# eriq-augustine/KB2E

Measured on AMD Instinct MI355X. Metric: training triples/sec (1/2/4/8 MI355X) + FB15k Hits@10(Filter), higher is better.
Workload: dtype f64

## Files before the change

kb2e_amd/csrc/kernels_transr_pipe.hpp:

```cpp
#pragma once

#include "kernels_transr_cons.hpp"
#include "kernels_transr_seq.hpp"

namespace kb2e {

constexpr int kPipeList = 1536;

template <typename T>
__host__ __device__ constexpr size_t pipe_lds(int n) {
    return sizeof(T) * ((size_t)rm_np(n) * rm_ld(n) + 5 * (size_t)kChainRows * rm_ld(n) +
                        3 * (size_t)kChainRows * (kChainRows + 1) + 4 * kChainRows + 4 * (size_t)rm_np(n)) +
           sizeof(int) * (size_t)(2 * kPipeList + kSeqMaxTiles + 1 + 8 + 2 * kChainRows);
}

template <typename T, int KS>
__global__ __launch_bounds__(kChainThreads) void transr_cons_pipe_kernel(RParArgs a, RParBufs<T> bf) {
    using M = Mfma16<T>;
    static_assert(sizeof(T) == 8, "the D-row / k-step identity below is the FP64 fragment layout");
    constexpr int NB = (4 * KS + 15) / 16;
    constexpr int NP = 16 * NB, L = NP + 2, R = kChainRows, LG = R + 1;
    constexpr int NH = 2 * KS;
    constexpr int NSW = (NB + 2) / 3;
    static_assert(2 * R * L >= NP * L, "the K0 image borrows the two P buffers");
    static_assert(NSW * KS <= 4 * KS, "the helpers' slices share the walk's K0 registers");
    const int t0 = a.batch_t0[a.batch], t1 = a.batch_t0[a.batch + 1];
    int g0, r;
    if (!chain_first_tile(a, t0, t1, g0, r)) return;
    const int n = a.n, ld = a.ld;
    const int w = threadIdx.x >> 6, l = lane_id(), kq = l >> 4, l16 = l & 15;
    const bool mine = w < NB;
    const int col = 16 * w + l16;
    const int hw = w - 1;
    const T lr = (T)a.lr;
    extern __shared__ __attribute__((aligned(16))) char smem[];
    T* Wc = (T*)smem;
    T* Abuf = Wc + NP * L;
    T* Pbuf = Abuf + 3 * R * L;
    T* Gbuf = Pbuf + 2 * R * L;
    T* Cx = Gbuf + 2 * R * LG;
    T* qpart = Cx + R * LG;
    T* rp = qpart + 4 * R;
    int* pe = (int*)(rp + 4 * NP);
    int* ps = pe + kPipeList;
    int* pre = ps + kPipeList;
    int* misc = pre + kSeqMaxTiles + 1;
    int* vlist = misc + 8;
    const long long ck0 = clock64();
    unsigned long long n_chunks = 0, n_vio = 0, n_rounds = 0, max_m = 0;
    __shared__ unsigned long long ph[16];
    if (threadIdx.x < 16) ph[threadIdx.x] = 0;
    long long tq = ck0;
    auto tick = [&](int k) {
        if (bf.stats && threadIdx.x == (k >= 12 || k == 5 ? 64u : 0u)) {
            const long long t = clock64();
            ph[k] += (unsigned long long)(t - tq);
            tq = t;
        }
    };

    for (int idx = threadIdx.x; idx < NP * NP; idx += kChainThreads) {
        const int j = idx / NP, i = idx % NP;
        Wc[j * L + i] = (j < n && i < n) ? bf.W[((int64_t)r * n + j) * ld + i] : T(0);
    }
    if (w == 0) {
        int run = 0;
        for (int m0 = 0;; m0 += kWave) {
            const int g = g0 + m0 + l;
            const uint64_t b = __ballot(t0 + g < t1 && a.td_r[t0 + g] == r);
            const int k = b == ~0ull ? kWave : __builtin_ctzll(~b);
            run += k;
            if (k < kWave) break;
        }
        const int c0 = bf.cnrows[g0] & 127;
        const int rel = c0 > 0 && bf.cpairs[(int64_t)g0 * 2 * kCPairs + kCPairs + c0 - 1] == -2;
        int kl = -1, gt = -1;
        for (int g = g0 + run - 1; g >= g0 && kl < 0; --g) {
            const int cs = a.td_cnt[t0 + g] & 255;
            const int kk = l < cs ? a.td_kk[(t0 + g) * 8 + l] : -1;
            const uint64_t b = __ballot(kk >= 0 && a.act[kk]);
            if (b) {
                kl = __shfl(kk, 63 - __builtin_clzll(b));
                gt = g;
            }
        }
        int ntail = 0;
        if (gt >= 0) {
            const int cp = bf.cnrows[gt] & 127;
            const int sl = l < cp ? bf.cpairs[(int64_t)gt * 2 * kCPairs + kCPairs + l] : -3;
            ntail = __builtin_popcountll(__ballot(sl >= 0 && (sl >> 1) == kl * 2 + 1));
        }
        if (l == 0) {
            misc[3] = rel;
            misc[4] = gt;
            misc[5] = run;
            misc[6] = ntail;
        }
    }
    __syncthreads();
    const int run = misc[5], has_rel = misc[3], g_tail = misc[4], n_tail = misc[6];
    T reg[4 * KS];
    {
        T* K0 = Pbuf;
        if (mine) {
#pragma unroll
            for (int ib = 0; ib < NB; ++ib) {
                typename M::acc_t acc = {T(0), T(0), T(0), T(0)};
                T av[KS], bv[KS];
#pragma unroll
                for (int s = 0; s < KS; ++s) {
                    av[s] = Wc[(4 * s + kq) * L + ib * 16 + l16];
                    bv[s] = Wc[(4 * s + kq) * L + col];
                }
#pragma unroll
                for (int s = 0; s < KS; ++s) acc = M::mma(av[s], bv[s], acc);
#pragma unroll
                for (int qq = 0; qq < 4; ++qq) K0[(ib * 16 + kq + 4 * qq) * L + col] = acc[qq];
            }
        }
        __syncthreads();
        if (w == 0) {
            const int cK = l < NP ? l : 0;
#pragma unroll
            for (int i = 0; i < 4 * KS; ++i) reg[i] = K0[i * L + cK];
        } else {
#pragma unroll
            for (int i = 0; i < 4 * KS; ++i) reg[i] = T(0);
#pragma unroll
            for (int si = 0; si < NSW; ++si) {
                const int cb = hw + 3 * si;
                if (cb < NB) {
#pragma unroll
                    for (int s = 0; s < KS; ++s) reg[si * KS + s] = Wc[(4 * s + kq) * L + cb * 16 + l16];
                }
            }
        }
        if (threadIdx.x == 0) {
            misc[5] = 0;
            misc[6] = -1;
            misc[7] = -1;
        }
        __syncthreads();
    }
    bool changed = false;
    int32_t* const vio = bf.vio + (int64_t)g0 * kCPairs;
    int nvt = 0;
    int pend_nv = 0, pend_par = 0, pend_pc = 0, pend_ka = 0;
    tick(0);

    auto gram_tile = [&](const T* Ar, const T* Bm, int rt, int cb, T* out, int ldo) {
        typename M::acc_t acc = {T(0), T(0), T(0), T(0)};
        T av[KS], bv[KS];
#pragma unroll
        for (int s = 0; s < KS; ++s) {
            av[s] = Ar[(rt * 16 + l16) * L + 4 * s + kq];
            bv[s] = Bm[(cb * 16 + l16) * L + 4 * s + kq];
        }
#pragma unroll
        for (int s = 0; s < KS; ++s) acc = M::mma(av[s], bv[s], acc);
#pragma unroll
        for (int q = 0; q < 4; ++q) out[(rt * 16 + kq + 4 * q) * ldo + cb * 16 + l16] = acc[q];
    };
    auto proj_tile = [&](const T* Ar, int rt, int si, T* out) {
        const int cb = hw + 3 * si;
        typename M::acc_t acc = {T(0), T(0), T(0), T(0)};
        T av[KS];
#pragma unroll
        for (int s = 0; s < KS; ++s) av[s] = Ar[(rt * 16 + l16) * L + 4 * s + kq];
#pragma unroll
        for (int s = 0; s < KS; ++s) acc = M::mma(av[s], reg[si * KS + s], acc);
#pragma unroll
        for (int q = 0; q < 4; ++q) out[(rt * 16 + kq + 4 * q) * L + cb * 16 + l16] = acc[q];
    };
    constexpr int kHT = kChainThreads - kWave;
    constexpr int kRowsPer = (R * NP + kHT - 1) / kHT;
    static_assert(kRowsPer <= 32, "rows_ok bits");
    const int ht = (int)threadIdx.x - kWave;
    T rows[kRowsPer];
    uint32_t rows_ok = 0;
    auto load_rows = [&](int b, int e) {
        if (w == 0) return;
        int ent[kRowsPer];
#pragma unroll
        for (int q = 0; q < kRowsPer; ++q) {
            const int f = b + (ht + q * kHT) / NP;
            ent[q] = pe[f < kPipeList ? f : kPipeList - 1];
        }
        rows_ok = 0;
#pragma unroll
        for (int q = 0; q < kRowsPer; ++q) {
            const int idx = ht + q * kHT;
            const int k = idx / NP, j = idx % NP;
            const bool ok = idx < R * NP && b + k < e && ent[q] >= 0 && j < n;
            rows[q] = bf.ent[ok ? (uint32_t)ent[q] * (uint32_t)ld + (uint32_t)j : 0u];
            rows_ok |= (ok ? 1u : 0u) << q;
        }
    };
    auto store_rows = [&](int slot) {
        if (w == 0) return;
#pragma unroll
        for (int q = 0; q < kRowsPer; ++q) {
            const int idx = ht + q * kHT;
            if (idx < R * NP) Abuf[slot * R * L + (idx / NP) * L + idx % NP] = ((rows_ok >> q) & 1) ? rows[q] : T(0);
        }
    };
    int hsync_target = 0;
    auto helper_sync = [&]() {
        hsync_target += kChainThreads / kWave - 1;
        if (l == 0 && !((bf.dbg & 32) && hw == 0))
            __hip_atomic_fetch_add(&misc[5], 1, __ATOMIC_RELEASE, __HIP_MEMORY_SCOPE_WORKGROUP);
        for (uint32_t sp = 0;
             __hip_atomic_load(&misc[5], __ATOMIC_ACQUIRE, __HIP_MEMORY_SCOPE_WORKGROUP) < hsync_target; ++sp) {
            if (sp > (1u << 22)) {
                if (l == 0) __hip_atomic_store(bf.err, 1u, __ATOMIC_RELAXED, __HIP_MEMORY_SCOPE_AGENT);
                break;
            }
            __builtin_amdgcn_s_sleep(1);
        }
    };
    auto correct_inc = [&](T* Pn, int cn, const T* Pc, const T* An, const T* Ac, const int* vl, int ck) {
        constexpr int NE = NP / 16, NPS = (R + 11) / 12;
        const int rs = ht >> 4, cb = (ht & 15) * NE;
        T x[NPS][NE];
#pragma unroll
        for (int p = 0; p < NPS; ++p) {
            const int j = rs + 12 * p;
#pragma unroll
            for (int u = 0; u < NE; ++u) x[p][u] = j < cn ? Pn[j * L + cb + u] : T(0);
        }
        int used = 0;
        for (uint32_t sp = 0;; ++sp) {
            const bool done = __hip_atomic_load(&misc[6], __ATOMIC_ACQUIRE, __HIP_MEMORY_SCOPE_WORKGROUP) == ck;
            const int pw = __hip_atomic_load(&misc[7], __ATOMIC_ACQUIRE, __HIP_MEMORY_SCOPE_WORKGROUP);
            const int avail = (pw >> 6) == ck ? (pw & 63) : 0;
            for (; used < avail; ++used) {
                const int v = vl[used];
                T gv[NE], av[NE], d[NPS];
#pragma unroll
                for (int u = 0; u < NE; ++u) {
                    gv[u] = Pc[v * L + cb + u];
                    av[u] = Ac[v * L + cb + u];
                }
#pragma unroll
                for (int p = 0; p < NPS; ++p) {
                    const int j = rs + 12 * p;
                    d[p] = T(0);
#pragma unroll
                    for (int u = 0; u < NE; ++u) d[p] = fma(j < R ? An[j * L + cb + u] : T(0), av[u], d[p]);
                }
                row16_sums<T, NPS>(d);
#pragma unroll
                for (int p = 0; p < NPS; ++p) {
                    const int j = rs + 12 * p;
                    if (j < cn) {
                        const T gl = -lr * d[p];
#pragma unroll
                        for (int u = 0; u < NE; ++u) x[p][u] = fma(gl, gv[u], x[p][u]);
                    }
                }
            }
            if (done) break;
            if (sp > (1u << 22)) {
                if (l == 0) __hip_atomic_store(bf.err, 1u, __ATOMIC_RELAXED, __HIP_MEMORY_SCOPE_AGENT);
                break;
            }
            __builtin_amdgcn_s_sleep(1);
        }
        T sq[NPS];
#pragma unroll
        for (int p = 0; p < NPS; ++p) {
            const int j = rs + 12 * p;
            sq[p] = T(0);
            if (j < cn) {
#pragma unroll
                for (int u = 0; u < NE; ++u) {
                    if (used) Pn[j * L + cb + u] = x[p][u];
                    sq[p] = fma(x[p][u], x[p][u], sq[p]);
                }
            }
        }
        row16_sums<T, NPS>(sq);
        if ((ht & 15) == 0) {
#pragma unroll
            for (int p = 0; p < NPS; ++p) {
                const int j = rs + 12 * p;
                if (j < R) {
                    qpart[j] = j < cn ? sq[p] : T(0);
                    for (int v = 1; v < NB; ++v) qpart[v * R + j] = T(0);
                }
            }
        }
    };
    auto correct_q = [&](T* Pn, int cn, int nv, const T* Pc, const int* vl) {
        constexpr int NE = NP / 8;
        const int j = threadIdx.x >> 3, cb = (threadIdx.x & 7) * NE;
        T sq = T(0);
        if (j < cn) {
            T x[NE];
#pragma unroll
            for (int u = 0; u < NE; ++u) x[u] = Pn[j * L + cb + u];
            for (int k = 0; k < nv; ++k) {
                const int v = vl[k];
                const T gl = -lr * Cx[j * LG + v];
#pragma unroll
                for (int u = 0; u < NE; ++u) x[u] = fma(gl, Pc[v * L + cb + u], x[u]);
            }
#pragma unroll
            for (int u = 0; u < NE; ++u) {
                if (nv) Pn[j * L + cb + u] = x[u];
                sq = fma(x[u], x[u], sq);
            }
        }
        sq += dpp_mov<0xB1>(sq);
        sq += dpp_mov<0x4E>(sq);
        sq += dpp_mov<0x141>(sq);
        if ((threadIdx.x & 7) == 0) {
            qpart[j] = j < cn ? sq : T(0);
            for (int v = 1; v < NB; ++v) qpart[v * R + j] = T(0);
        }
    };
    auto apply_pending = [&]() {
        if (w == 0 || pend_nv == 0) return;
        const T* Pp = Pbuf + pend_pc * R * L;
        const T* Ap = Abuf + pend_ka * R * L;
        const int* vl = vlist + pend_par * R;
        const int vmine = l < pend_nv ? vl[l] : 0;
        T an[KS], gn[NSW];
        auto ldv = [&](int k) {
            const int v = __builtin_amdgcn_readlane(vmine, k);
#pragma unroll
            for (int s = 0; s < KS; ++s) an[s] = Ap[v * L + 4 * s + kq];
#pragma unroll
            for (int si = 0; si < NSW; ++si) {
                const int cb = hw + 3 * si;
                gn[si] = cb < NB ? -lr * Pp[v * L + cb * 16 + l16] : T(0);
            }
        };
        const int nvu = (bf.dbg & 16) ? 0 : pend_nv;
        if (nvu > 0) ldv(0);
        for (int k = 0; k < nvu; ++k) {
            T ac[KS], gc[NSW];
#pragma unroll
            for (int s = 0; s < KS; ++s) ac[s] = an[s];
#pragma unroll
            for (int si = 0; si < NSW; ++si) gc[si] = gn[si];
            if (k + 1 < nvu) ldv(k + 1);
#pragma unroll
            for (int si = 0; si < NSW; ++si)
                if (hw + 3 * si < NB) {
#pragma unroll
                    for (int s = 0; s < KS; ++s) reg[si * KS + s] = fma(ac[s], gc[si], reg[si * KS + s]);
                }
        }
    };
    auto renorm = [&] {
        if (w > 0) {
#pragma unroll
            for (int si = 0; si < NSW; ++si) {
                const int cb = hw + 3 * si;
#pragma unroll
                for (int s = 0; s < KS; ++s) {
                    T x[1] = {reg[si * KS + s] * reg[si * KS + s]};
                    row16_sums<T, 1>(x);
                    if (cb < NB && l16 == 0) rp[cb * NP + 4 * s + kq] = x[0];
                }
            }
        }
        __syncthreads();
        if (w > 0) {
#pragma unroll
            for (int si = 0; si < NSW; ++si) {
                if (hw + 3 * si >= NB) continue;
#pragma unroll
                for (int s = 0; s < KS; ++s) {
                    const int jr = 4 * s + kq;
                    T ss = rp[jr];
                    for (int v = 1; v < NB; ++v) ss += rp[v * NP + jr];
                    if (jr < n) reg[si * KS + s] = reg[si * KS + s] / sqrt(ss);
                }
            }
        }
        __syncthreads();
    };
    auto fresh = [&](const T* A, int cc, T* P, T* G) {
        const int nrt = cc > 16 ? 2 : 1;
        if (w > 0) {
#pragma unroll
            for (int si = 0; si < NSW; ++si)
                if (hw + 3 * si < NB)
                    for (int rt = 0; rt < nrt; ++rt) proj_tile(A, rt, si, P);
        } else {
            for (int gi = 0; gi < (nrt == 2 ? 3 : 1); ++gi) gram_tile(A, A, gi == 0 ? 0 : 1, gi == 2 ? 1 : 0, G, LG);
        }
        __syncthreads();
        correct_q(P, cc, 0, nullptr, vlist);
        __syncthreads();
    };

    const int tile_cap = bf.chain_tiles >= 1 && bf.chain_tiles < kSeqMaxTiles ? bf.chain_tiles : kSeqMaxTiles;
    const int list_cap = bf.chain_list >= 64 && bf.chain_list < kPipeList ? bf.chain_list : kPipeList;
    int pc = 0;
    int par = 0;
    for (int gw = g0; gw < g0 + run || gw == g0;) {
        if (w == 0) {
            const int nt = g0 + run - gw < tile_cap ? g0 + run - gw : tile_cap;
            int carry = 0, fit = 0;
            for (int m0 = 0; m0 < nt; m0 += kWave) {
                const int g = m0 + l;
                int c = g < nt ? (bf.cnrows[gw + g] & 127) : 0;
                if (gw + g == g0 && has_rel) c -= 1;
                int x = c;
#pragma unroll
                for (int s = 1; s < kWave; s <<= 1) {
                    const int y = __shfl_up(x, s);
                    if (l >= s) x += y;
                }
                if (g < nt) pre[g] = carry + x - c;
                fit += __builtin_popcountll(__ballot(g < nt && carry + x <= list_cap - 1));
                carry += __shfl(x, kWave - 1);
            }
            if (l == 0) {
                if (fit == nt) pre[nt] = carry;
                misc[0] = fit;
            }
        }
        __syncthreads();
        const int ntile = misc[0];
        const bool last = gw + ntile == g0 + run || (g_tail >= 0 && gw + ntile > g_tail);
        const int ntp = pre[ntile];
        const int npairs = ntp + (last && has_rel ? 1 : 0);
        const int tail_start = last && g_tail >= gw ? ntp - n_tail : npairs;
        for (int f = threadIdx.x; f < npairs; f += kChainThreads) {
            int e = r, sl = -2;
            if (f < ntp) {
                int lo = 0, hi = ntile - 1;
                while (lo < hi) {
                    const int mid = (lo + hi + 1) >> 1;
                    if (pre[mid] <= f) lo = mid;
                    else hi = mid - 1;
                }
                const int32_t* cp = bf.cpairs + (int64_t)(gw + lo) * 2 * kCPairs;
                e = cp[f - pre[lo]];
                sl = cp[kCPairs + f - pre[lo]];
            }
            pe[f] = e;
            ps[f] = sl;
        }
        auto chunk_end = [&](int b) {
            return b < tail_start ? (b + R < tail_start ? b + R : tail_start) : npairs;
        };
        __syncthreads();
        if (npairs > 0) {
            const int e0 = chunk_end(0);
            const int e1 = e0 < npairs ? chunk_end(e0) : e0;
            load_rows(0, e0);
            store_rows(0);
            load_rows(e0, e1);
            store_rows(1);
            load_rows(e1, e1 < npairs ? chunk_end(e1) : e1);
            if (tail_start == 0 && changed) renorm();
            __syncthreads();
            pc = 0;
            fresh(Abuf, e0, Pbuf, Gbuf);
        }
        int ka = 0;
        for (int base = 0; base < npairs;) {
            const int nbase = chunk_end(base);
            const int cc = nbase - base;
            const int nb2 = nbase < npairs ? chunk_end(nbase) : nbase;
            const int cn = nb2 - nbase;
            const T* A = Abuf + ka * R * L;
            const T* An = Abuf + (ka == 2 ? 0 : ka + 1) * R * L;
            T* P = Pbuf + pc * R * L;
            T* Pn = Pbuf + (pc ^ 1) * R * L;
            T* Gm = Gbuf + pc * R * LG;
            T* Gn = Gbuf + (pc ^ 1) * R * LG;
            int* vl = vlist + par * R;
            const int ck = (int)n_chunks;
            ++n_chunks;
            tick(1);
            if (w == 0) {
                const int j = l & (R - 1);
                T q = T(0);
                if (j < cc) {
                    q = qpart[j];
                    for (int v = 1; v < NB; ++v) q += qpart[v * R + j];
                }
                uint32_t vmask = 0;
                int npub = 0;
                if (__ballot(j < cc && q > T(1)) != 0) {
                    const T aaj = Gm[j * LG + j];
                    const int c0 = (l >> 5) * NH;
                    T x[NH];
#pragma unroll
                    for (int u = 0; u < NH; ++u) x[u] = P[j * L + c0 + u];
                    int cursor = 0;
                    const T eps = T(2) * lr;
                    for (;;) {
                        const uint64_t cand = __ballot(l < R && j < cc && j >= cursor && q > T(1));
                        if (!cand) break;
                        const int v = __builtin_ctzll(cand);
                        const int c = l;
                        const T pp = readlane_f(q, v);
                        const T aa = readlane_f(aaj, v);
                        const T cjv = Gm[j * LG + v];
                        const int slv = ps[base + v];
                        if (j == v) {
#pragma unroll
                            for (int u = 0; u < NH; ++u) P[v * L + c0 + u] = x[u];
                        }
                        tick(4);
                        const T pv = c < NP ? P[v * L + c] : T(0);
                        T vv4[4] = {T(0), T(0), T(0), T(0)};
#pragma unroll
                        for (int t = 0; t < KS; ++t)
#pragma unroll
                            for (int u = 0; u < 4; ++u) vv4[u] = fma(P[v * L + 4 * t + u], reg[4 * t + u], vv4[u]);
                        const T Vc = c < n ? (vv4[0] + vv4[1]) + (vv4[2] + vv4[3]) : T(0);
                        tick(7);
                        T s2[2] = {pv * Vc, Vc * Vc};
                        T rpp = __builtin_amdgcn_rcp(pp);
                        rpp = fma(fma(-pp, rpp, T(1)), rpp, rpp);
                        rpp = fma(fma(-pp, rpp, T(1)), rpp, rpp);
                        wave_sums<T, 2>(s2);
                        tick(8);
                        const T pV = s2[0], VV = s2[1];
                        const T pvd = pV + aa * pp, vvd = VV + T(2) * aa * pV + aa * aa * pp;
                        const T kappa = pvd * rpp;
                        const T w2t = vvd - kappa * pvd;
                        const T w2 = w2t > T(0) ? w2t : T(0);
                        const T rho = T(1) - eps * kappa;
                        T S0, S1;
                        const int m = transr_rounds_violator4(pp, w2, eps, rho, S0, S1);
                        n_rounds += (unsigned long long)m;
                        max_m = max_m > (unsigned long long)m ? max_m : (unsigned long long)m;
                        const T cpf = T(2) * (S0 + eps * S1 * kappa), cvf = T(2) * eps * S1;
                        const T g = c < n ? cpf * pv - cvf * (Vc + aa * pv) : T(0);
                        tick(9);
                        if (c < NP) P[v * L + c] = g;
                        {
                            T* dst = slv >= 0 ? bf.pair + (int64_t)slv * ld : bf.relpair + (int64_t)r * ld;
                            if (c < n) dst[c] = g;
                            if (l == 0) vio[nvt + npub] = slv;
                        }
                        tick(10);
                        const bool upd = j > v && j < cc;
                        T qh = T(0);
                        if (upd) {
                            const T gl = -lr * cjv;
                            T s4[4] = {T(0), T(0), T(0), T(0)};
#pragma unroll
                            for (int u = 0; u < NH; ++u) {
                                x[u] = fma(gl, P[v * L + c0 + u], x[u]);
                                s4[u & 3] = fma(x[u], x[u], s4[u & 3]);
                            }
                            qh = (s4[0] + s4[1]) + (s4[2] + s4[3]);
                        }
                        {
                            const T tot = pair_sum32(qh);
                            if (upd) q = tot;
                        }
                        if (l == 0) {
                            vl[npub] = v;
                            __hip_atomic_store(&misc[7], (ck << 6) | (npub + 1), __ATOMIC_RELEASE,
                                               __HIP_MEMORY_SCOPE_WORKGROUP);
                        }
                        ++npub;
                        vmask |= 1u << v;
                        cursor = v + 1;
                        ++n_vio;
                        tick(11);
                    }
                }
                if (l < cc) {
                    const int sl = ps[base + l];
                    const bool vio_l = (vmask >> l) & 1;
                    if (sl >= 0) bf.pflag[sl] = vio_l ? 1 : 0;
                    else if (vio_l) bf.relpair_stamp[r] = bf.stamp;
                }
                if (l == 0) {
                    misc[1 + 2 * par] = (int)vmask;
                    misc[2 + 2 * par] = npub;
                    __hip_atomic_store(&misc[6], ck, __ATOMIC_RELEASE, __HIP_MEMORY_SCOPE_WORKGROUP);
                }
                tick(2);
            } else {
                apply_pending();
                tick(12);
                if (cn > 0) {
                    const int nrt = cn > 16 ? 2 : 1, crt = cc > 16 ? 2 : 1;
#pragma unroll
                    for (int si = 0; si < NSW; ++si)
                        if (hw + 3 * si < NB)
                            for (int rt = 0; rt < nrt; ++rt) proj_tile(An, rt, si, Pn);
                    const int ng = nrt == 2 ? 3 : 1;
                    int load[3];
#pragma unroll
                    for (int h = 0; h < 3; ++h) load[h] = nrt * ((NB - h + 2) / 3);
                    for (int tl = 0; tl < ng; ++tl) {
                        int best = 0;
#pragma unroll
                        for (int h = 1; h < 3; ++h) best = load[h] < load[best] ? h : best;
                        ++load[best];
                        if (best == hw) gram_tile(An, An, tl == 0 ? 0 : 1, tl == 2 ? 1 : 0, Gn, LG);
                    }
                    (void)crt;
                }
                tick(13);
                helper_sync();
                tick(14);
                if (nb2 < npairs || cn > 0) {
                    store_rows(ka == 0 ? 2 : ka - 1);
                    const int n3 = nb2 < npairs ? chunk_end(nb2) : nb2;
                    load_rows(n3, n3 < npairs ? chunk_end(n3) : n3);
                }
                if (cn > 0) correct_inc(Pn, cn, P, An, A, vl, ck);
                tick(15);
            }
            __syncthreads();
            tick(w == 0 ? 3 : 5);
            const uint32_t vmask = (uint32_t)misc[1 + 2 * par];
            const int nv = misc[2 + 2 * par];
            pend_nv = nv;
            pend_par = par;
            pend_pc = pc;
            pend_ka = ka;
            nvt += nv;
            if (vmask) changed = true;
            const bool restart = nbase == tail_start && changed && cn > 0;
            tick(6);
            if (restart) {
                apply_pending();
                pend_nv = 0;
                __syncthreads();
                renorm();
                fresh(An, cn, Pn, Gn);
            }
            pc ^= 1;
            par ^= 1;
            ka = ka == 2 ? 0 : ka + 1;
            base = nbase;
        }
        apply_pending();
        pend_nv = 0;
        __syncthreads();
        gw += ntile;
        if (last || gw >= g0 + run) break;
    }
    if (w > 0) {
#pragma unroll
        for (int si = 0; si < NSW; ++si) {
            const int cb = hw + 3 * si;
            if (cb < NB) {
#pragma unroll
                for (int s = 0; s < KS; ++s) Wc[(4 * s + kq) * L + cb * 16 + l16] = reg[si * KS + s];
            }
        }
    }
    __syncthreads();
    if (mine && col < n)
        for (int jj = 0; jj < n; ++jj) bf.W[((int64_t)r * n + jj) * ld + col] = Wc[jj * L + col];
    chain_records<T, NP, L>(a, bf, r, vio, nvt, Wc, Pbuf, 2 * R * L);
    if (bf.stats) {
        if (threadIdx.x == 0) {
            const unsigned long long cyc = (unsigned long long)(clock64() - ck0);
            atomicAdd(&g_seq_stats[0], 1ull);
            atomicAdd(&g_seq_stats[1], n_chunks);
            atomicAdd(&g_seq_stats[2], n_vio);
            atomicAdd(&g_seq_stats[3], n_rounds);
            atomicAdd(&g_seq_stats[4], cyc);
            atomicMax(&g_seq_stats[5], cyc);
            atomicMax(&g_seq_stats[6], n_chunks);
            atomicMax(&g_seq_stats[7], max_m);
            for (int k = 0; k < 16; ++k) atomicAdd(&g_seq_stats[8 + k], ph[k]);
            if (n_chunks >= 20) {
                for (int k = 0; k < 16; ++k) atomicAdd(&g_seq_stats[24 + k], ph[k]);
                atomicAdd(&g_seq_stats[40], n_chunks);
                atomicAdd(&g_seq_stats[41], 1ull);
                atomicAdd(&g_seq_stats[42], n_vio);
            }
        }
    }
}

}
```

kb2e_amd/csrc/transr_cons.hip:

```cpp
#include "transr_cons.hpp"

#include <algorithm>
#include <cstring>
#include <stdexcept>
#include <string>
#include <utility>

#include "hip_util.hpp"
#include "kernels_transr_cons.hpp"
#include "kernels_transr_seq.hpp"
#include "kernels_transr_chainw.hpp"
#include "kernels_transr_chainwp.hpp"
#include "kernels_transr_chaing.hpp"
#include "kernels_transr_pipe.hpp"
#include "kernels_transr_wave.hpp"

namespace kb2e {

namespace {

enum Kind { kCons, kGrad, kProj };

int chain_grid(const RParArgs& a) { return a.nrel > 0 ? a.nrel : 1; }

template <typename T, int KS>
const void* fn_at(Kind k) {
    return k == kCons ? (const void*)transr_cons_wave_kernel<T, KS>
           : k == kGrad ? (const void*)transr_grad_wave_kernel<T, KS>
                        : (const void*)transr_proj_wave_kernel<T, KS>;
}

template <typename T, int... KS>
const void* fn_table(Kind k, int ks, std::integer_sequence<int, KS...>) {
    const void* tab[] = {fn_at<T, KS + 1>(k)...};
    return tab[ks - 1];
}

template <typename T>
const void* kernel_fn(Kind k, int n) {
    if (!cons_wave_supported(n)) throw std::runtime_error("TransR wave kernels: n > 64");
    return fn_table<T>(k, cons_live_steps<T>(n), std::make_integer_sequence<int, 16>{});
}

template <typename T>
const void* cons_fn(int n) {
    return kernel_fn<T>(kCons, n);
}

template <int... KS>
const void* pipe_table(int ks, std::integer_sequence<int, KS...>) {
    const void* tab[] = {(const void*)transr_cons_pipe_kernel<double, KS + 1>...};
    return tab[ks - 1];
}

const void* pipe_fn(int n) {
    if (!cons_wave_supported(n)) throw std::runtime_error("transRNorm pipelined chain kernel: n > 64");
    return pipe_table((n + 3) / 4, std::make_integer_sequence<int, 16>{});
}

const void* chainw_fn(int n) {
    switch (wide_nb(n)) {
        case 1: return (const void*)transr_cons_chain_wide_kernel<1>;
        case 2: return (const void*)transr_cons_chain_wide_kernel<2>;
        case 3: return (const void*)transr_cons_chain_wide_kernel<3>;
        case 4: return (const void*)transr_cons_chain_wide_kernel<4>;
        case 5: return (const void*)transr_cons_chain_wide_kernel<5>;
        case 6: return (const void*)transr_cons_chain_wide_kernel<6>;
        case 7: return (const void*)transr_cons_chain_wide_kernel<7>;
    }
    throw std::runtime_error("transRNorm wide chain kernel: n > 112");
}

const void* chainwp_fn(int n) {
    switch (wp_ks(n)) {
        case 18: return (const void*)transr_cons_chain_wpipe_kernel<18>;
        case 20: return (const void*)transr_cons_chain_wpipe_kernel<20>;
        case 22: return (const void*)transr_cons_chain_wpipe_kernel<22>;
        case 24: return (const void*)transr_cons_chain_wpipe_kernel<24>;
        case 25: return (const void*)transr_cons_chain_wpipe_kernel<25>;
    }
    throw std::runtime_error("transRNorm pipelined wide chain kernel: no instantiation");
}

bool use_wpipe(int n) {
    const char* e = getenv("KB2E_RPAR_CHAIN");
    return n > 64 && n <= kWPMaxN && !(e && std::string(e) == "lockstep");
}

}

size_t cons_seq_setup(int n) {
    const size_t lds = pipe_lds<double>(n);
    HIPCHK(hipFuncSetAttribute(pipe_fn(n), hipFuncAttributeMaxDynamicSharedMemorySize, (int)lds));
    return lds;
}

void cons_seq_launch(const RParArgs& a, const RParBufs<double>& bf, size_t lds, hipStream_t stream) {
    RParArgs aa = a;
    RParBufs<double> bb = bf;
    void* args[] = {&aa, &bb};
    HIPCHK(hipLaunchKernel(pipe_fn(a.n), dim3(chain_grid(a)), dim3(kChainThreads), args, lds, stream));
}

bool cons_chainw_supported(int n) { return n >= 1 && n <= kWideMaxN; }

size_t cons_chainw_setup(int n) {
    HIPCHK(hipFuncSetAttribute((const void*)transr_cons_da_rel_kernel, hipFuncAttributeMaxDynamicSharedMemorySize,
                               (int)da_rel_lds(n)));
    const bool wp = use_wpipe(n);
    const size_t lds = wp ? chainwp_lds(n) : chainw_lds(n);
    HIPCHK(hipFuncSetAttribute(wp ? chainwp_fn(n) : chainw_fn(n), hipFuncAttributeMaxDynamicSharedMemorySize,
                               (int)lds));
    return lds;
}

bool cons_chainw_pipelined(int n) { return use_wpipe(n); }

void cons_chainw_launch(const RParArgs& a, const RParBufs<double>& bf, size_t lds, hipStream_t stream) {
    RParArgs aa = a;
    RParBufs<double> bb = bf;
    void* args[] = {&aa, &bb};
    const int grid = chain_grid(a);
    if (use_wpipe(a.n)) {
        HIPCHK(hipLaunchKernel(chainwp_fn(a.n), dim3(grid), dim3(kWPThreads), args, lds, stream));
    } else {
        HIPCHK(hipLaunchKernel(chainw_fn(a.n), dim3(grid), dim3(kWideThreads), args, lds, stream));
        HIPCHK(hipLaunchKernel((const void*)transr_cons_da_rel_kernel, dim3(grid), dim3(kDaRelThreads), args,
                               da_rel_lds(a.n), stream));
    }
}

bool cons_wave_supported(int n) { return n >= 1 && n <= 64; }

size_t cons_wave_setup(int n, int St, int esize) {
    const size_t lds = esize == 8 ? rcons_lds<double>(n, St) : rcons_lds<float>(n, St);
    HIPCHK(hipFuncSetAttribute(esize == 8 ? cons_fn<double>(n) : cons_fn<float>(n),
                               hipFuncAttributeMaxDynamicSharedMemorySize, (int)lds));
    return lds;
}

template <typename T>
void cons_wave_launch(const RParArgs& a, const RParBufs<T>& bf, int grid, size_t lds, hipStream_t stream) {
    RParArgs aa = a;
    RParBufs<T> bb = bf;
    void* args[] = {&aa, &bb};
    HIPCHK(hipLaunchKernel(cons_fn<T>(a.n), dim3(grid), dim3(kConsWaves * kWave), args, lds, stream));
}

template <typename T>
void grad_wave_launch(const RParArgs& a, const RParBufs<T>& bf, int grid, hipStream_t stream) {
    RParArgs aa = a;
    RParBufs<T> bb = bf;
    void* args[] = {&aa, &bb};
    HIPCHK(hipLaunchKernel(kernel_fn<T>(kGrad, a.n), dim3(grid), dim3(kConsWaves * kWave), args, 0, stream));
}

template <typename T>
void proj_wave_launch(const RParArgs& a, const RParBufs<T>& bf, int grid, hipStream_t stream) {
    RParArgs aa = a;
    RParBufs<T> bb = bf;
    void* args[] = {&aa, &bb};
    const size_t lds = sizeof(T) * (size_t)proj_wave_rows<T>(cons_live_steps<T>(a.n)) * rm_ld(a.n);
    HIPCHK(hipLaunchKernel(kernel_fn<T>(kProj, a.n), dim3(grid), dim3(kProjWaves * kWave), args, lds, stream));
}

bool cons_chaing_supported(int n) { return n >= 1 && n <= kGenMaxN; }

size_t cons_chaing_setup(int n, int esize) {
    const size_t lds = chaing_lds(n);
    HIPCHK(hipFuncSetAttribute(esize == 8 ? (const void*)transr_cons_chain_gen_kernel<double>
                                          : (const void*)transr_cons_chain_gen_kernel<float>,
                               hipFuncAttributeMaxDynamicSharedMemorySize, (int)lds));
    return lds;
}

template <typename T>
void cons_chaing_launch(const RParArgs& a, const RParBufs<T>& bf, size_t lds, hipStream_t stream) {
    RParArgs aa = a;
    RParBufs<T> bb = bf;
    void* args[] = {&aa, &bb};
    HIPCHK(hipLaunchKernel((const void*)transr_cons_chain_gen_kernel<T>, dim3(chain_grid(a)), dim3(kGenThreads), args,
                           lds, stream));
}
template void cons_chaing_launch<double>(const RParArgs&, const RParBufs<double>&, size_t, hipStream_t);
template void cons_chaing_launch<float>(const RParArgs&, const RParBufs<float>&, size_t, hipStream_t);

template void proj_wave_launch<double>(const RParArgs&, const RParBufs<double>&, int, hipStream_t);
template void proj_wave_launch<float>(const RParArgs&, const RParBufs<float>&, int, hipStream_t);

template void grad_wave_launch<double>(const RParArgs&, const RParBufs<double>&, int, hipStream_t);
template void grad_wave_launch<float>(const RParArgs&, const RParBufs<float>&, int, hipStream_t);

template void cons_wave_launch<double>(const RParArgs&, const RParBufs<double>&, int, size_t, hipStream_t);
template void cons_wave_launch<float>(const RParArgs&, const RParBufs<float>&, int, size_t, hipStream_t);

void cons_seq_take_stats(unsigned long long (&st)[64]) {
    HIPCHK(hipMemcpyFromSymbol(st, HIP_SYMBOL(g_seq_stats), sizeof(st)));
    unsigned long long z[64] = {};
    HIPCHK(hipMemcpyToSymbol(HIP_SYMBOL(g_seq_stats), z, sizeof(z)));
}

void cons_wave_take_stats(unsigned long long (&st)[16]) {
    unsigned long long mine[16];
    HIPCHK(hipMemcpyFromSymbol(mine, HIP_SYMBOL(g_cons_stats), sizeof(mine)));
    for (int k = 0; k < 16; ++k) st[k] = (k == 2 || k == 6) ? std::max(st[k], mine[k]) : st[k] + mine[k];
    std::memset(mine, 0, sizeof(mine));
    HIPCHK(hipMemcpyToSymbol(HIP_SYMBOL(g_cons_stats), mine, sizeof(mine)));
}

}
```

Before: 8.311 million.

## Offload violator output stores to helper waves and compile out stats

Adds a compile-time STATS template parameter so the clock64 and counter instrumentation disappears from the production kernel. The per-violator global stores of the gradient row, the violator record and the pflag/relpair stamps move off the serial walk wave into the helper waves' correction loop (renamed chunk_outputs). The helpers now run that loop even when no next chunk exists. The walk's P-row dot product is software-pipelined into grouped loads with sched_barriers, and the diagonal row write is replaced by a post-update store. This shortens the critical serial path, at the cost of more complex helper synchronisation and more register pressure.

Result: faster. 8.760 million, median of 6 (+5.4%).

```diff
diff --git a/kb2e_amd/csrc/kernels_transr_pipe.hpp b/kb2e_amd/csrc/kernels_transr_pipe.hpp
--- a/kb2e_amd/csrc/kernels_transr_pipe.hpp
+++ b/kb2e_amd/csrc/kernels_transr_pipe.hpp
@@ -14,7 +14,7 @@
            sizeof(int) * (size_t)(2 * kPipeList + kSeqMaxTiles + 1 + 8 + 2 * kChainRows);
 }
 
-template <typename T, int KS>
+template <typename T, int KS, bool STATS>
 __global__ __launch_bounds__(kChainThreads) void transr_cons_pipe_kernel(RParArgs a, RParBufs<T> bf) {
     using M = Mfma16<T>;
     static_assert(sizeof(T) == 8, "the D-row / k-step identity below is the FP64 fragment layout");
@@ -46,16 +46,19 @@
     int* pre = ps + kPipeList;
     int* misc = pre + kSeqMaxTiles + 1;
     int* vlist = misc + 8;
-    const long long ck0 = clock64();
-    unsigned long long n_chunks = 0, n_vio = 0, n_rounds = 0, max_m = 0;
-    __shared__ unsigned long long ph[16];
-    if (threadIdx.x < 16) ph[threadIdx.x] = 0;
+    const long long ck0 = STATS ? clock64() : 0;
+    int n_chunks = 0;
+    unsigned long long n_vio = 0, n_rounds = 0, max_m = 0;
+    __shared__ unsigned long long ph[STATS ? 16 : 1];
+    if (STATS && threadIdx.x < 16) ph[threadIdx.x] = 0;
     long long tq = ck0;
     auto tick = [&](int k) {
-        if (bf.stats && threadIdx.x == (k >= 12 || k == 5 ? 64u : 0u)) {
-            const long long t = clock64();
-            ph[k] += (unsigned long long)(t - tq);
-            tq = t;
+        if constexpr (STATS) {
+            if (threadIdx.x == (k >= 12 || k == 5 ? 64u : 0u)) {
+                const long long t = clock64();
+                ph[k] += (unsigned long long)(t - tq);
+                tq = t;
+            }
         }
     };
 
@@ -218,7 +221,8 @@
             __builtin_amdgcn_s_sleep(1);
         }
     };
-    auto correct_inc = [&](T* Pn, int cn, const T* Pc, const T* An, const T* Ac, const int* vl, int ck) {
+    auto chunk_outputs = [&](T* Pn, int cn, const T* Pc, const T* An, const T* Ac, const int* vl, int ck, int base,
+                             int cc, int vpar) {
         constexpr int NE = NP / 16, NPS = (R + 11) / 12;
         const int rs = ht >> 4, cb = (ht & 15) * NE;
         T x[NPS][NE];
@@ -235,37 +239,56 @@
             const int avail = (pw >> 6) == ck ? (pw & 63) : 0;
             for (; used < avail; ++used) {
                 const int v = vl[used];
+                const int slv = ps[base + v];
                 T gv[NE], av[NE], d[NPS];
 #pragma unroll
                 for (int u = 0; u < NE; ++u) {
                     gv[u] = Pc[v * L + cb + u];
                     av[u] = Ac[v * L + cb + u];
                 }
-#pragma unroll
-                for (int p = 0; p < NPS; ++p) {
-                    const int j = rs + 12 * p;
-                    d[p] = T(0);
-#pragma unroll
-                    for (int u = 0; u < NE; ++u) d[p] = fma(j < R ? An[j * L + cb + u] : T(0), av[u], d[p]);
-                }
-                row16_sums<T, NPS>(d);
-#pragma unroll
-                for (int p = 0; p < NPS; ++p) {
-                    const int j = rs + 12 * p;
-                    if (j < cn) {
-                        const T gl = -lr * d[p];
-#pragma unroll
-                        for (int u = 0; u < NE; ++u) x[p][u] = fma(gl, gv[u], x[p][u]);
+                if (cn > 0) {
+#pragma unroll
+                    for (int p = 0; p < NPS; ++p) {
+                        const int j = rs + 12 * p;
+                        d[p] = T(0);
+#pragma unroll
+                        for (int u = 0; u < NE; ++u) d[p] = fma(j < R ? An[j * L + cb + u] : T(0), av[u], d[p]);
                     }
-                }
-            }
-            if (done) break;
+                    row16_sums<T, NPS>(d);
+#pragma unroll
+                    for (int p = 0; p < NPS; ++p) {
+                        const int j = rs + 12 * p;
+                        if (j < cn) {
+                            const T gl = -lr * d[p];
+#pragma unroll
+                            for (int u = 0; u < NE; ++u) x[p][u] = fma(gl, gv[u], x[p][u]);
+                        }
+                    }
+                }
+                if (rs == 0) {
+                    T* dst = slv >= 0 ? bf.pair + (int64_t)slv * ld : bf.relpair + (int64_t)r * ld;
+#pragma unroll
+                    for (int u = 0; u < NE; ++u)
+                        if (cb + u < n) dst[cb + u] = gv[u];
+                    if (ht == 0) vio[nvt + used] = slv;
+                }
+            }
+            if (done) {
+                if (ht < cc) {
+                    const int sl = ps[base + ht];
+                    const bool vio_l = ((uint32_t)misc[1 + 2 * vpar] >> ht) & 1;
+                    if (sl >= 0) bf.pflag[sl] = vio_l ? 1 : 0;
+                    else if (vio_l) bf.relpair_stamp[r] = bf.stamp;
+                }
+                break;
+            }
             if (sp > (1u << 22)) {
                 if (l == 0) __hip_atomic_store(bf.err, 1u, __ATOMIC_RELAXED, __HIP_MEMORY_SCOPE_AGENT);
                 break;
             }
             __builtin_amdgcn_s_sleep(1);
         }
+        if (cn == 0) return;
         T sq[NPS];
 #pragma unroll
         for (int p = 0; p < NPS; ++p) {
@@ -476,7 +499,7 @@
             T* Gm = Gbuf + pc * R * LG;
             T* Gn = Gbuf + (pc ^ 1) * R * LG;
             int* vl = vlist + par * R;
-            const int ck = (int)n_chunks;
+            const int ck = n_chunks;
             ++n_chunks;
             tick(1);
             if (w == 0) {
@@ -504,18 +527,35 @@
                         const T pp = readlane_f(q, v);
                         const T aa = readlane_f(aaj, v);
                         const T cjv = Gm[j * LG + v];
-                        const int slv = ps[base + v];
-                        if (j == v) {
-#pragma unroll
-                            for (int u = 0; u < NH; ++u) P[v * L + c0 + u] = x[u];
+                        tick(4);
+                        T vv4[4] = {T(0), T(0), T(0), T(0)};
+                        constexpr int NG = 6;
+                        T pr[4 * KS];
+                        auto v_load = [&](int g) {
+#pragma unroll
+                            for (int t = g * KS / NG; t < (g + 1) * KS / NG; ++t)
+#pragma unroll
+                                for (int u = 0; u < 4; ++u) pr[4 * t + u] = P[v * L + 4 * t + u];
+                        };
+                        auto v_fma = [&](int g) {
+#pragma unroll
+                            for (int t = g * KS / NG; t < (g + 1) * KS / NG; ++t)
+#pragma unroll
+                                for (int u = 0; u < 4; ++u) vv4[u] = fma(pr[4 * t + u], reg[4 * t + u], vv4[u]);
+                        };
+                        v_load(0);
+                        v_load(1);
+                        const T pv = c < NP ? P[v * L + c] : T(0);
+                        __builtin_amdgcn_sched_barrier(0);
+#pragma unroll
+                        for (int g = 0; g < NG; ++g) {
+                            v_fma(g);
+                            if (g + 2 < NG) {
+                                __builtin_amdgcn_sched_barrier(0);
+                                v_load(g + 2);
+                                __builtin_amdgcn_sched_barrier(0);
+                            }
                         }
-                        tick(4);
-                        const T pv = c < NP ? P[v * L + c] : T(0);
-                        T vv4[4] = {T(0), T(0), T(0), T(0)};
-#pragma unroll
-                        for (int t = 0; t < KS; ++t)
-#pragma unroll
-                            for (int u = 0; u < 4; ++u) vv4[u] = fma(P[v * L + 4 * t + u], reg[4 * t + u], vv4[u]);
                         const T Vc = c < n ? (vv4[0] + vv4[1]) + (vv4[2] + vv4[3]) : T(0);
                         tick(7);
                         T s2[2] = {pv * Vc, Vc * Vc};
@@ -532,28 +572,31 @@
                         const T rho = T(1) - eps * kappa;
                         T S0, S1;
                         const int m = transr_rounds_violator4(pp, w2, eps, rho, S0, S1);
-                        n_rounds += (unsigned long long)m;
-                        max_m = max_m > (unsigned long long)m ? max_m : (unsigned long long)m;
+                        if constexpr (STATS) {
+                            n_rounds += (unsigned long long)m;
+                            max_m = max_m > (unsigned long long)m ? max_m : (unsigned long long)m;
+                        }
                         const T cpf = T(2) * (S0 + eps * S1 * kappa), cvf = T(2) * eps * S1;
                         const T g = c < n ? cpf * pv - cvf * (Vc + aa * pv) : T(0);
                         tick(9);
                         if (c < NP) P[v * L + c] = g;
-                        {
-                            T* dst = slv >= 0 ? bf.pair + (int64_t)slv * ld : bf.relpair + (int64_t)r * ld;
-                            if (c < n) dst[c] = g;
-                            if (l == 0) vio[nvt + npub] = slv;
-                        }
                         tick(10);
                         const bool upd = j > v && j < cc;
                         T qh = T(0);
                         if (upd) {
                             const T gl = -lr * cjv;
                             T s4[4] = {T(0), T(0), T(0), T(0)};
+                            T gr[NH];
+#pragma unroll
+                            for (int u = 0; u < NH; ++u) gr[u] = P[v * L + c0 + u];
+                            __builtin_amdgcn_sched_barrier(0);
 #pragma unroll
                             for (int u = 0; u < NH; ++u) {
-                                x[u] = fma(gl, P[v * L + c0 + u], x[u]);
+                                x[u] = fma(gl, gr[u], x[u]);
                                 s4[u & 3] = fma(x[u], x[u], s4[u & 3]);
                             }
+#pragma unroll
+                            for (int u = 0; u < NH; ++u) P[j * L + c0 + u] = x[u];
                             qh = (s4[0] + s4[1]) + (s4[2] + s4[3]);
                         }
                         {
@@ -568,15 +611,9 @@
                         ++npub;
                         vmask |= 1u << v;
                         cursor = v + 1;
-                        ++n_vio;
+                        if constexpr (STATS) ++n_vio;
                         tick(11);
                     }
-                }
-                if (l < cc) {
-                    const int sl = ps[base + l];
-                    const bool vio_l = (vmask >> l) & 1;
-                    if (sl >= 0) bf.pflag[sl] = vio_l ? 1 : 0;
-                    else if (vio_l) bf.relpair_stamp[r] = bf.stamp;
                 }
                 if (l == 0) {
                     misc[1 + 2 * par] = (int)vmask;
@@ -614,7 +651,7 @@
                     const int n3 = nb2 < npairs ? chunk_end(nb2) : nb2;
                     load_rows(n3, n3 < npairs ? chunk_end(n3) : n3);
                 }
-                if (cn > 0) correct_inc(Pn, cn, P, An, A, vl, ck);
+                chunk_outputs(Pn, cn, P, An, A, vl, ck, base, cc, par);
                 tick(15);
             }
             __syncthreads();
@@ -661,21 +698,21 @@
     if (mine && col < n)
         for (int jj = 0; jj < n; ++jj) bf.W[((int64_t)r * n + jj) * ld + col] = Wc[jj * L + col];
     chain_records<T, NP, L>(a, bf, r, vio, nvt, Wc, Pbuf, 2 * R * L);
-    if (bf.stats) {
+    if constexpr (STATS) {
         if (threadIdx.x == 0) {
             const unsigned long long cyc = (unsigned long long)(clock64() - ck0);
             atomicAdd(&g_seq_stats[0], 1ull);
-            atomicAdd(&g_seq_stats[1], n_chunks);
+            atomicAdd(&g_seq_stats[1], (unsigned long long)n_chunks);
             atomicAdd(&g_seq_stats[2], n_vio);
             atomicAdd(&g_seq_stats[3], n_rounds);
             atomicAdd(&g_seq_stats[4], cyc);
             atomicMax(&g_seq_stats[5], cyc);
-            atomicMax(&g_seq_stats[6], n_chunks);
+            atomicMax(&g_seq_stats[6], (unsigned long long)n_chunks);
             atomicMax(&g_seq_stats[7], max_m);
             for (int k = 0; k < 16; ++k) atomicAdd(&g_seq_stats[8 + k], ph[k]);
-            if (n_chunks >= 20) {
+            if (n_chunks >= 12) {
                 for (int k = 0; k < 16; ++k) atomicAdd(&g_seq_stats[24 + k], ph[k]);
-                atomicAdd(&g_seq_stats[40], n_chunks);
+                atomicAdd(&g_seq_stats[40], (unsigned long long)n_chunks);
                 atomicAdd(&g_seq_stats[41], 1ull);
                 atomicAdd(&g_seq_stats[42], n_vio);
             }
diff --git a/kb2e_amd/csrc/transr_cons.hip b/kb2e_amd/csrc/transr_cons.hip
--- a/kb2e_amd/csrc/transr_cons.hip
+++ b/kb2e_amd/csrc/transr_cons.hip
@@ -47,15 +47,16 @@
     return kernel_fn<T>(kCons, n);
 }
 
-template <int... KS>
+template <bool STATS, int... KS>
 const void* pipe_table(int ks, std::integer_sequence<int, KS...>) {
-    const void* tab[] = {(const void*)transr_cons_pipe_kernel<double, KS + 1>...};
+    const void* tab[] = {(const void*)transr_cons_pipe_kernel<double, KS + 1, STATS>...};
     return tab[ks - 1];
 }
 
-const void* pipe_fn(int n) {
+const void* pipe_fn(int n, bool stats) {
     if (!cons_wave_supported(n)) throw std::runtime_error("transRNorm pipelined chain kernel: n > 64");
-    return pipe_table((n + 3) / 4, std::make_integer_sequence<int, 16>{});
+    const auto seq = std::make_integer_sequence<int, 16>{};
+    return stats ? pipe_table<true>((n + 3) / 4, seq) : pipe_table<false>((n + 3) / 4, seq);
 }
 
 const void* chainw_fn(int n) {
@@ -91,7 +92,8 @@
 
 size_t cons_seq_setup(int n) {
     const size_t lds = pipe_lds<double>(n);
-    HIPCHK(hipFuncSetAttribute(pipe_fn(n), hipFuncAttributeMaxDynamicSharedMemorySize, (int)lds));
+    for (const bool stats : {false, true})
+        HIPCHK(hipFuncSetAttribute(pipe_fn(n, stats), hipFuncAttributeMaxDynamicSharedMemorySize, (int)lds));
     return lds;
 }
 
@@ -99,7 +101,7 @@
     RParArgs aa = a;
     RParBufs<double> bb = bf;
     void* args[] = {&aa, &bb};
-    HIPCHK(hipLaunchKernel(pipe_fn(a.n), dim3(chain_grid(a)), dim3(kChainThreads), args, lds, stream));
+    HIPCHK(hipLaunchKernel(pipe_fn(a.n, bf.stats != 0), dim3(chain_grid(a)), dim3(kChainThreads), args, lds, stream));
 }
 
 bool cons_chainw_supported(int n) { return n >= 1 && n <= kWideMaxN; }
```
